# NVlabs/FasterViT

Hardware: AMD Instinct MI355X
Metric: images/sec FasterViT-0 224x224 inference, bs=256/GPU (higher is better)
Workload: dtype f16; 1 GPU; faster_vit_0_224 inference, 224x224, batch 256/GPU, synthetic weights (tests/synth.py init family); global_batch=256, parallelism=dp1 (independent shards, no data-path collective), hat_operands=f16, streams=1

## Files before the change

fastervit_amd/csrc/fvit_api.hip:

```cpp
#include <stdarg.h>
#include <stdlib.h>
#include <string.h>

#include <algorithm>
#include <map>
#include <mutex>
#include <string>
#include <vector>

#include "fvit_common.h"

namespace fvit {

static thread_local char g_err[512] = "";

void set_error(const char* fmt, ...) {
    va_list ap;
    va_start(ap, fmt);
    vsnprintf(g_err, sizeof(g_err), fmt, ap);
    va_end(ap);
}

int check_launch(const char* what) {
    hipError_t e = hipGetLastError();
// ... 170 lines not shown
                            const void* w_fc2_frag, const float* b_fc2, const float* gamma2, float eps) {
    return {dtype, X, rowsA, src_idx, add, R, batch, G, heads, C, hidden, ln1_w, ln1_b, w_qkv_frag, b_qkv_heads, w_proj_frag,
            b_proj, gamma1, bias, scale, ln2_w, ln2_b, w_fc1_frag, b_fc1, w_fc2_frag, b_fc2, gamma2, eps};
}

enum class CarrierRoute {
    NONE,
    FUSED_CT,
    ATTNBLK,
    LNGEMM_CHAIN,
    CHAIN,
};
enum class WinAttnRoute {
    WINBLK,
    ATTNBLK,
    LNGEMM_PREADDED,
    CHAIN,
};
enum class MlpRoute {
    WINMLP,
    MLP_FUSED,
    LNGEMM_CHAIN,
    CHAIN,
};

struct BlockRoute {
    CarrierRoute carrier = CarrierRoute::NONE;
    MlpRoute carrier_mlp = MlpRoute::CHAIN;
    WinAttnRoute window_attn = WinAttnRoute::CHAIN;
    MlpRoute window_mlp = MlpRoute::CHAIN;
    bool preadd_eligible = false;
    const float* pe_next = nullptr;
    int win_blk_split = 1, win_mlp_split = 1;
    RowMap entry_map;
    const float* entry_ct = nullptr;
    RowMap exit_map;
    const float* exit_ln_w = nullptr;
    const float* exit_ln_b = nullptr;
    float exit_eps = 0.f;
};

struct RouteKnobs {
    const int ln_gemm = tune_get("ln_gemm", 0), ln_gemm_max_rows = tune_get("ln_gemm_max_rows", 16384);
    const int attn_fused = tune_get("attn_fused", 1), attn_fused_x2 = tune_get("attn_fused_x2", 1);
    const int attn_fused_min_rows = tune_get("attn_fused_min_rows", 16384), attn_fused512_min_rows = tune_get("attn_fused512_min_rows", 1 << 30);
    const int mlp_fused = tune_get("mlp_fused", 1);
    const int mlp_fused_min_rows = tune_get("mlp_fused_min_rows", 16384), mlp_fused512_min_rows = tune_get("mlp_fused512_min_rows", 1 << 30);
    const int win_mlp = tune_get("win_mlp", 1), win_mlp256 = tune_get("win_mlp256", 2), win_mlp_split = tune_get("win_mlp_split", 1);
    const int win_fused = tune_get("win_fused", 1), win_fused256 = tune_get("win_fused256", 0), win_blk_split = tune_get("win_blk_split", 1);
    const int ct_fused = tune_get("ct_fused", 1), pe_preadd = tune_get("pe_preadd", 1);
    const int stage_entry_fused = tune_get("stage_entry_fused", 1), stage_exit_fused = tune_get("stage_exit_fused", 1);
};

static BlockRoute choose_route(const FvitStageDesc& d, const StageLayout& L, const FvitBlockWeights& w, const RouteKnobs& k) {
    const int T = d.weight_terms;
    auto ln_gemm_ok = [&](int N, int ldo, int64_t rows) {
        return T == 1 && ln_gemm_supported(d.C, N, L.ldn, ldo) && k.ln_gemm && rows <= k.ln_gemm_max_rows;
    };
    auto attnblk = [&](const FvitAttnWeights& a, int S, int64_t rows) {
        const bool terms_ok = T == 1 || (T == 2 && d.C == 256 && S > 48 && k.attn_fused_x2);
        return terms_ok && a.w_qkv_frag && a.b_qkv_heads && a.w_proj_frag && d.dpad == 32 && d.C / d.heads == 32 && attnblk_supported(d.C, d.heads, S) &&
               rows >= (d.C == 256 ? k.attn_fused_min_rows : k.attn_fused512_min_rows) && k.attn_fused;
    };
    auto mlp = [&](const FvitMlpWeights& m, int64_t rows) {
        const bool frags = m.w_fc1_frag && m.w_fc2_frag;
        if (T <= 2 && frags && winmlp_supported(d.C, d.hidden) && (d.C == 512 ? k.win_mlp != 0 : rows >= k.mlp_fused_min_rows && k.win_mlp256 != 0))
            return MlpRoute::WINMLP;
        if (T == 1 && frags && mlp_fused_supported(d.C, d.hidden) && rows >= (d.C == 256 ? k.mlp_fused_min_rows : k.mlp_fused512_min_rows) && k.mlp_fused)
            return MlpRoute::MLP_FUSED;
        return ln_gemm_ok(d.hidden, L.ldh, rows) ? MlpRoute::LNGEMM_CHAIN : MlpRoute::CHAIN;
    };

    BlockRoute r;
    r.win_blk_split = k.win_blk_split;
    r.win_mlp_split = k.win_mlp_split;
    if (d.hier) {
        const FvitAttnWeights& a = w.hat_attn;
        if (T <= 2 && ctblk_supported(d.C, d.heads, L.G, d.hidden) && d.dpad == 32 && a.w_qkv_frag && a.b_qkv_heads && a.w_proj_frag && a.bias &&
            w.hat_mlp.w_fc1_frag && w.hat_mlp.w_fc2_frag && k.ct_fused)
            r.carrier = CarrierRoute::FUSED_CT;
        else if (attnblk(a, L.G, L.Mc))
            r.carrier = CarrierRoute::ATTNBLK;
        else
            r.carrier = ln_gemm_ok(L.ldqkv, L.ldqkv, L.Mc) ? CarrierRoute::LNGEMM_CHAIN : CarrierRoute::CHAIN;
        r.carrier_mlp = mlp(w.hat_mlp, L.Mc);
    }
    const FvitAttnWeights& a = w.attn;
    if (T <= 2 && (T == 1 || d.C == 512) && winblk_supported(d.C, d.heads, L.S) && d.dpad == 32 && a.w_qkv_frag && a.b_qkv_heads && a.w_proj_frag && a.bias &&
        (d.C == 512 ? k.win_fused != 0 : k.win_fused256 != 0))
        r.window_attn = WinAttnRoute::WINBLK;
    else if (attnblk(a, L.S, L.Mx))
        r.window_attn = WinAttnRoute::ATTNBLK;
    r.window_mlp = mlp(w.mlp, L.Mx);
    r.preadd_eligible = !d.hier && r.window_attn == WinAttnRoute::CHAIN && (r.window_mlp == MlpRoute::CHAIN || r.window_mlp == MlpRoute::LNGEMM_CHAIN) &&
                        ln_gemm_ok(L.ldqkv, L.ldqkv, L.Mx) && k.pe_preadd;
    return r;
}

struct Branch {
    float* x;
    int64_t rows;
    void *xn, *qkv, *ao, *h;
    int nwin, S;
};

static LnCall ln_call(const FvitStageDesc& d, const StageLayout& L, const float* ln_w, const float* ln_b, const float* src, int64_t rows, void* n_out) {
    LnCall ln = {d.operand_dtype, src, 0, nullptr, 0, nullptr, nullptr, nullptr, nullptr, n_out, L.at * L.ldn, ln_w, ln_b, 1e-5f, (int)rows, 1, d.C};
    if (L.at == 2) ln.lo_off = L.ldn;
// ... 79 lines not shown
static AttnBlkCall window_attnblk_call(const FvitStageDesc& d, const StageLayout& L, const FvitBlockWeights& w, const FvitStageTables& t, float* X, float* R) {
    const FvitAttnWeights& a = w.attn;
    AttnBlkCall ab = attnblk_call(d.operand_dtype, X, L.rpi, R, L.G, (d.hier ? t.ln1_src : nullptr), t.ln1_add, w.pe_x, a.ln_w, a.ln_b, 1e-5f, L.rpi,
                                  a.w_qkv_frag, a.b_qkv_heads, a.w_proj_frag, a.b_proj, a.gamma, a.bias, X, d.batch * L.nW, L.S, d.heads, d.C, L.scale);
    ab.terms = d.weight_terms;
    return ab;
}

static MlpFusedCall window_mlp_call(const FvitStageDesc& d, const StageLayout& L, const FvitMlpWeights& w, float* X) {
    MlpFusedCall mc = mlp_fused_call(d.operand_dtype, X, (int)L.Mx, d.C, d.hidden, w.ln_w, w.ln_b, 1e-5f, w.w_fc1_frag, w.b_fc1, w.w_fc2_frag, w.b_fc2, w.gamma);
    mc.terms = d.weight_terms;
    return mc;
}

static RowMap row_map(const FvitStageDesc& d, const StageLayout& L, const FvitMapView& m) {
    RowMap r;
    r.data = m.data; r.stride_b = m.stride_b; r.stride_h = m.stride_h; r.stride_w = m.stride_w; r.bf16 = m.dtype == FVIT_BF16;
    r.S = L.S; r.ncw = L.ncw; r.ws = d.ws; r.nwx = d.Wp / d.ws; r.nw = L.nW;
    return r;
}
static bool map_16bit_cl(const FvitMapView& m, int align_bytes) {
    return (m.dtype == FVIT_F16 || m.dtype == FVIT_BF16) && m.stride_c == 1 && ((uintptr_t)m.data % align_bytes) == 0 && (m.stride_b * 2) % align_bytes == 0 &&
           (m.stride_h * 2) % align_bytes == 0 && (m.stride_w * 2) % align_bytes == 0;
}

static AttnBlkCall window_winblk_call(const FvitStageDesc& d, const StageLayout& L, const BlockRoute& r, const FvitBlockWeights& w, const FvitStageTables& t,
                                      float* X, float* R, char* ws) {
    AttnBlkCall ab = window_attnblk_call(d, L, w, t, X, R);
    if (L.off_SLAB) {
        ab.slab = (float*)(ws + L.off_SLAB);
        ab.counters = (int*)(ws + L.off_CNT);
        ab.nsplit = r.win_blk_split;
    }
    return ab;
}

static void choose_stage_boundaries(const FvitStageDesc& d, const StageLayout& L, const FvitBlockWeights* blocks, const FvitStageTables& t, const FvitMapView& in,
                                    const float* ct_init, const FvitMapView* out, const FvitStageTail* tail, bool prop, const ReverseCall& rc,
                                    const RouteKnobs& k, char* ws, std::vector<BlockRoute>& routes) {
    if (d.depth <= 0 || d.H != d.Hp || d.W != d.Wp || prop) return;
    for (int i = 0; i < d.depth; ++i)
        if (blocks[i].attn.gamma || blocks[i].mlp.gamma || (d.hier && (blocks[i].hat_attn.gamma || blocks[i].hat_mlp.gamma))) return;
    float* X = (float*)(ws + L.off_X);
    float* R = (float*)(ws + L.off_R);
    BlockRoute& first = routes[0];
    if (k.stage_entry_fused && map_16bit_cl(in, 8) && d.C % 4 == 0 && d.weight_terms <= 2) {
        bool ok = false;
        if (first.window_attn == WinAttnRoute::ATTNBLK) ok = attnblk_map_source_supported(window_attnblk_call(d, L, blocks[0], t, X, R));
        else if (first.window_attn == WinAttnRoute::WINBLK) ok = winblk_map_source_supported(window_winblk_call(d, L, first, blocks[0], t, X, R, ws));
        if (ok) {
            first.entry_map = row_map(d, L, in);
            if (first.carrier == CarrierRoute::FUSED_CT) first.entry_ct = ct_init;
        }
    }
    BlockRoute& last = routes[d.depth - 1];
    if (k.stage_exit_fused && tail && tail->ln_w && out && reverse_ln_supported(rc) && last.window_mlp == MlpRoute::WINMLP &&
        winmlp_exit_supported(window_mlp_call(d, L, blocks[d.depth - 1].mlp, X))) {
        last.exit_map = row_map(d, L, *out);
        last.exit_ln_w = tail->ln_w;
        last.exit_ln_b = tail->ln_b;
        last.exit_eps = tail->ln_eps;
    }
}

static int run_block(const FvitStageDesc& d, const StageLayout& L, const BlockRoute& r, const FvitBlockWeights& w, const FvitStageTables& t,
                     char* ws, hipStream_t st) {
// ... 385 lines not shown

int fvit_win_mlp_fused_terms(int32_t operand_dtype, float* x, int32_t M, int32_t C, int32_t hidden, const float* ln_w, const float* ln_b,
                             float eps, const void* w_fc1_frag, const float* b_fc1, const void* w_fc2_frag, const float* b_fc2,
                             const float* gamma, int32_t terms, fvit_stream_t stream) {
    MlpFusedCall mc = mlp_fused_call(operand_dtype, x, M, C, hidden, ln_w, ln_b, eps, w_fc1_frag, b_fc1, w_fc2_frag, b_fc2, gamma);
    mc.terms = terms;
    return launch_winmlp(mc, (hipStream_t)stream);
}

size_t fvit_win_mlp_split_bytes(int32_t M, int32_t C, int32_t nsplit) { return winmlp_split_slab_bytes(M, C, nsplit); }

int fvit_win_mlp_fused_split(int32_t operand_dtype, float* x, int32_t M, int32_t C, int32_t hidden, const float* ln_w, const float* ln_b,
                             float eps, const void* w_fc1_frag, const float* b_fc1, const void* w_fc2_frag, const float* b_fc2,
                             const float* gamma, int32_t terms, float* slab, int32_t* counters, int32_t nsplit, fvit_stream_t stream) {
    if (C != 512 || (nsplit != 1 && nsplit != 2) || (nsplit > 1 && (!slab || !counters))) {
        set_error("win_mlp_fused_split: C = %d nsplit = %d (C must be 512, nsplit 1 / 2 with scratch)", C, nsplit);
        return FVIT_EINVAL;
    }
    MlpFusedCall mc = mlp_fused_call(operand_dtype, x, M, C, hidden, ln_w, ln_b, eps, w_fc1_frag, b_fc1, w_fc2_frag, b_fc2, gamma);
    mc.terms = terms;
    mc.slab = slab; mc.counters = counters; mc.nsplit = nsplit;
    return launch_winmlp(mc, (hipStream_t)stream);
}

int fvit_win_block_supported(int32_t C, int32_t heads, int32_t S) { return winblk_supported(C, heads, S) ? 1 : 0; }

int fvit_win_block_fused(int32_t operand_dtype, const float* srcA, int32_t rowsA, const float* srcB, int32_t rowsB, const int32_t* src_idx,
                         const int32_t* add_idx, const float* add, const float* ln_w, const float* ln_b, float eps,
                         int32_t rows_per_image, const void* w_qkv_frag, const float* b_qkv_heads, const void* w_proj_frag,
                         const float* b_proj, const float* gamma, const float* bias, float* x_out, int32_t nwin, int32_t S,
                         int32_t heads, int32_t C, float scale, fvit_stream_t stream) {
    AttnBlkCall ab = attnblk_call(operand_dtype, srcA, rowsA, srcB, rowsB, src_idx, add_idx, add, ln_w, ln_b, eps, rows_per_image, w_qkv_frag,
                                  b_qkv_heads, w_proj_frag, b_proj, gamma, bias, x_out, nwin, S, heads, C, scale);
    return launch_winblk(ab, (hipStream_t)stream);
}

#ifdef FVIT_DIAG
int fvit_debug_win_mlp_timeline(float* x, int32_t M, int32_t C, int32_t hidden, const float* ln_w, const float* ln_b, float eps,
                                const void* w_fc1_frag, const float* b_fc1, const void* w_fc2_frag, const float* b_fc2, const float* gamma,
                                void* stamps, fvit_stream_t stream) {
    if (!stamps) { set_error("debug_win_mlp_timeline: null stamp buffer"); return FVIT_EINVAL; }
    MlpFusedCall mc = mlp_fused_call(FVIT_F16, x, M, C, hidden, ln_w, ln_b, eps, w_fc1_frag, b_fc1, w_fc2_frag, b_fc2, gamma);
    mc.ts = stamps;
    return launch_winmlp(mc, (hipStream_t)stream);
}
#endif

int fvit_win_block_fused_split(int32_t operand_dtype, const float* srcA, int32_t rowsA, const float* srcB, int32_t rowsB, const int32_t* src_idx,
                               const int32_t* add_idx, const float* add, const float* ln_w, const float* ln_b, float eps,
                               int32_t rows_per_image, const void* w_qkv_frag, const float* b_qkv_heads, const void* w_proj_frag,
                               const float* b_proj, const float* gamma, const float* bias, float* x_out, int32_t nwin, int32_t S,
                               int32_t heads, int32_t C, float scale, float* slab, int32_t* counters, int32_t nsplit, fvit_stream_t stream) {
    if (C != 512 || (nsplit != 1 && nsplit != 2) || (nsplit > 1 && (!slab || !counters))) {
        set_error("win_block_fused_split: C = %d nsplit = %d (C must be 512, nsplit 1 / 2 with scratch)", C, nsplit);
        return FVIT_EINVAL;
    }
    AttnBlkCall ab = attnblk_call(operand_dtype, srcA, rowsA, srcB, rowsB, src_idx, add_idx, add, ln_w, ln_b, eps, rows_per_image, w_qkv_frag,
                                  b_qkv_heads, w_proj_frag, b_proj, gamma, bias, x_out, nwin, S, heads, C, scale);
    ab.slab = slab; ab.counters = counters; ab.nsplit = nsplit;
    return launch_winblk(ab, (hipStream_t)stream);
}

int fvit_win_block_fused_terms(int32_t operand_dtype, const float* srcA, int32_t rowsA, const float* srcB, int32_t rowsB, const int32_t* src_idx,
                               const int32_t* add_idx, const float* add, const float* ln_w, const float* ln_b, float eps,
                               int32_t rows_per_image, const void* w_qkv_frag, const float* b_qkv_heads, const void* w_proj_frag,
                               const float* b_proj, const float* gamma, const float* bias, float* x_out, int32_t nwin, int32_t S,
                               int32_t heads, int32_t C, float scale, int32_t terms, fvit_stream_t stream) {
    AttnBlkCall ab = attnblk_call(operand_dtype, srcA, rowsA, srcB, rowsB, src_idx, add_idx, add, ln_w, ln_b, eps, rows_per_image, w_qkv_frag,
                                  b_qkv_heads, w_proj_frag, b_proj, gamma, bias, x_out, nwin, S, heads, C, scale);
    ab.terms = terms;
    return launch_winblk(ab, (hipStream_t)stream);
}

int fvit_attn_block_fused_terms(int32_t operand_dtype, const float* srcA, int32_t rowsA, const float* srcB, int32_t rowsB, const int32_t* src_idx,
                                const int32_t* add_idx, const float* add, const float* ln_w, const float* ln_b, float eps,
                                int32_t rows_per_image, const void* w_qkv_frag, const float* b_qkv_heads, const void* w_proj_frag,
                                const float* b_proj, const float* gamma, const float* bias, float* x_out, int32_t nwin, int32_t S,
                                int32_t heads, int32_t C, float scale, int32_t terms, fvit_stream_t stream) {
    AttnBlkCall ab = attnblk_call(operand_dtype, srcA, rowsA, srcB, rowsB, src_idx, add_idx, add, ln_w, ln_b, eps, rows_per_image, w_qkv_frag,
                                  b_qkv_heads, w_proj_frag, b_proj, gamma, bias, x_out, nwin, S, heads, C, scale);
    ab.terms = terms;
    return launch_attnblk(ab, (hipStream_t)stream);
}

int fvit_ct_block_supported(int32_t C, int32_t heads, int32_t G, int32_t hidden) { return ctblk_supported(C, heads, G, hidden) ? 1 : 0; }

int fvit_ct_block_fused(int32_t operand_dtype, const float* X, int32_t rowsA, const int32_t* src_idx, const float* add, float* R,
                        int32_t batch, int32_t G, int32_t heads, int32_t C, int32_t hidden, const float* ln1_w, const float* ln1_b,
                        const void* w_qkv_frag, const float* b_qkv_heads, const void* w_proj_frag, const float* b_proj, const float* gamma1,
                        const float* bias, float scale, const float* ln2_w, const float* ln2_b, const void* w_fc1_frag, const float* b_fc1,
                        const void* w_fc2_frag, const float* b_fc2, const float* gamma2, float eps, fvit_stream_t stream) {
    CtBlkCall cb = ctblk_call(operand_dtype, X, rowsA, src_idx, add, R, batch, G, heads, C, hidden, ln1_w, ln1_b, w_qkv_frag, b_qkv_heads, w_proj_frag,
                              b_proj, gamma1, bias, scale, ln2_w, ln2_b, w_fc1_frag, b_fc1, w_fc2_frag, b_fc2, gamma2, eps);
    return launch_ctblk(cb, (hipStream_t)stream);
}

int fvit_ct_block_fused_terms(int32_t operand_dtype, const float* X, int32_t rowsA, const int32_t* src_idx, const float* add, float* R,
                              int32_t batch, int32_t G, int32_t heads, int32_t C, int32_t hidden, const float* ln1_w, const float* ln1_b,
                              const void* w_qkv_frag, const float* b_qkv_heads, const void* w_proj_frag, const float* b_proj, const float* gamma1,
                              const float* bias, float scale, const float* ln2_w, const float* ln2_b, const void* w_fc1_frag, const float* b_fc1,
                              const void* w_fc2_frag, const float* b_fc2, const float* gamma2, float eps, int32_t terms, fvit_stream_t stream) {
    CtBlkCall cb = ctblk_call(operand_dtype, X, rowsA, src_idx, add, R, batch, G, heads, C, hidden, ln1_w, ln1_b, w_qkv_frag, b_qkv_heads, w_proj_frag,
                              b_proj, gamma1, bias, scale, ln2_w, ln2_b, w_fc1_frag, b_fc1, w_fc2_frag, b_fc2, gamma2, eps);
// ... 96 lines not shown
```

fastervit_amd/csrc/fvit_common.h:

```cpp
#pragma once
#include <hip/hip_runtime.h>
#include <stdint.h>
#include <atomic>
#include <mutex>
#include <stdio.h>

#include "../../include/fvit_hip.h"

namespace fvit {

typedef _Float16 h8 __attribute__((ext_vector_type(8)));
typedef _Float16 h4 __attribute__((ext_vector_type(4)));
typedef __bf16 b8 __attribute__((ext_vector_type(8)));
typedef __bf16 b4 __attribute__((ext_vector_type(4)));
typedef float f4 __attribute__((ext_vector_type(4)));

template <typename T> struct Op16;
template <> struct Op16<_Float16> {
    typedef h8 v8;
    typedef h4 v4;
    static __device__ __forceinline__ f4 mfma(v8 a, v8 b, f4 c) {
        return __builtin_amdgcn_mfma_f32_16x16x32_f16(a, b, c, 0, 0, 0);
    }
};
// ... 330 lines not shown
bool winmlp_exit_supported(const MlpFusedCall& c);
size_t winmlp_split_slab_bytes(int64_t M, int C, int nsplit);
bool mlp_fused_supported(int C, int hidden);
int launch_mlp_fused(const MlpFusedCall& c, hipStream_t stream);
bool winmlp_supported(int C, int hidden);
int launch_winmlp(const MlpFusedCall& c, hipStream_t stream);

struct AttnBlkCall {
    int dtype;
    const float* srcA;
    int rowsA;
    const float* srcB;
    int rowsB;
    const int32_t* src_idx;
    const int32_t* add_idx;
    const float* add;
    const float* ln_w;
    const float* ln_b;
    float eps;
    int rows_per_image;
    const void* wqkv_f;
    const float* bqkv;
    const void* wproj_f;
    const float* bproj;
    const float* gamma;
    const float* bias;
    float* x_out;
    int nwin, S, heads, C;
    float scale;
    float* slab = nullptr;
    int* counters = nullptr;
    int nsplit = 1;
    int terms = 1;
    void* ts = nullptr;
    RowMap map;
};
bool attnblk_supported(int C, int heads, int S);
bool attnblk_map_source_supported(const AttnBlkCall& c);
bool winblk_map_source_supported(const AttnBlkCall& c);
int launch_attnblk(const AttnBlkCall& c, hipStream_t stream);
bool attnblk2_supported(int C, int heads, int S);
int launch_attnblk2(const AttnBlkCall& c, hipStream_t stream);
bool winblk_supported(int C, int heads, int S);
int launch_winblk(const AttnBlkCall& c, hipStream_t stream);
struct AttnCall {
    int dtype;
    const void* qkv;
    int ldq;
    void* out;
    int ldo;
    const float* bias;
    int nwin, S, heads, dpad;
    float scale;
    const float* rel_table;
    int rel_w, rel_ng;
    int d;
    int q_lo_off = 0, o_lo_off = 0;
    const void* drop_mask = nullptr;
};
bool attention_dense(int S, int dpad);
int launch_attention(const AttnCall& c, hipStream_t stream);
int launch_attention_long(const AttnCall& c, hipStream_t stream);

struct LnCall {
    int dtype;
    const float* srcA;
// ... 81 lines not shown
```

fastervit_amd/csrc/fvit_winblk.hip:

```cpp
#include "fvit_common.h"

namespace fvit {

namespace {

struct WinBlkParams {
    const float* srcA;
    const float* srcB;
    const int32_t* src_idx;
    const int32_t* add_idx;
    const float* add;
    const float* ln_w;
    const float* ln_b;
    float eps;
    int rowsA, rowsB, rows_per_image;
    const void* wqkv_f;
    const float* bqkv;
    const void* wproj_f;
    const float* bproj;
    const float* gamma;
    const float* bias;
    float* x_out;
    int nwin, S;
    float scale;
    float* slab;
    int* counters;
    RowMap map;
};

template <int CC, int NSPLIT>
constexpr int winblk_lds_bytes() { return 4 * (CC / 32) * 1024 + 4 * (CC / 32 / NSPLIT) * 1024 + (CC / 32) * 96 * 4; }

template <typename T, int CC, int NWV, int NSPLIT = 1, int WT = 1, bool MAPSRC = false>
__device__ __forceinline__ void winblk_body(const WinBlkParams& p, char* const smem, const int blk) {
    typedef typename Op16<T>::v8 v8;
    constexpr int C = CC, KK = C / 32, CB = C / 16, HEADS = C / 32, NW = NWV, NRB = 4, SP = 64;
    constexpr int HW = HEADS / NSPLIT;
    constexpr int NH = HW / NW;
    static_assert(HW == NH * NW && NH >= 1 && CB == 4 * NW, "heads split evenly over the waves; four output channel blocks per wave");
    constexpr int KQ = KK * WT, PW = HW * WT;
    constexpr int SPH = KQ + 4;
    constexpr size_t QKV_IMG = (size_t)3 * C * C * 2, PROJ_IMG = (size_t)C * C * 2;
    constexpr int DEPTH = 2;
    constexpr int OFF_O = NRB * KK * 1024;
    constexpr int OFF_BQ = OFF_O + NRB * HW * 1024;
    static_assert(OFF_BQ + HEADS * 96 * 4 == winblk_lds_bytes<CC, NSPLIT>(), "LDS layout");
    float* bqs = (float*)(smem + OFF_BQ);

    const int tid = threadIdx.x;
    const int lane = tid & 63;
    const int wave = __builtin_amdgcn_readfirstlane(tid >> 6);
    const int g = lane >> 4, s = lane & 15;
    const int lane16 = lane * 16;
    int win = blk, sp = 0;
    if constexpr (NSPLIT > 1) {
        const int xcd = blk & 7, j = blk >> 3;
        win = (j / NSPLIT) * 8 + xcd;
        sp = j % NSPLIT;
        if (win >= p.nwin) return;
    }
    const int h0 = sp * HW;

    const char* Wq = (const char*)p.wqkv_f + lane16;
    const char* Wp = (const char*)p.wproj_f + lane16;
    const char* Bz = (const char*)p.bias + (s * SP + g * 4) * 4;
    v8 ring[DEPTH][6];
    auto load_qkv = [&](int slot, int h, int u) {
// ... 275 lines not shown
            const char* mpx = nullptr;
            if (p.src_idx) {
                const int si = p.src_idx[pr];
                src = si >= 0 ? p.srcA + ((size_t)b * p.rowsA + si) * C : p.srcB + ((size_t)b * p.rowsB + (-si - 1)) * C;
                if constexpr (MAPSRC) {
                    if (si >= 0) mpx = rowmap_px(p.map, (int64_t)b * p.rowsA + si);
                }
            } else {
                src = p.srcA + (size_t)row * C;
                if constexpr (MAPSRC) mpx = rowmap_px(p.map, row);
            }
            const int ai = p.add ? (p.add_idx ? p.add_idx[pr] : pr) : -1;
            float* px = p.x_out + (size_t)row * C + c0;
            f4 xm[4];
            if constexpr (MAPSRC) {
                if (mpx) rowmap_load_row(xm, mpx, p.map.bf16, [&](int q) { return c0 + q * 4; });
            }
#pragma unroll
            for (int q = 0; q < 4; ++q) {
                f4 xv;
                if (MAPSRC && mpx) xv = xm[q];
                else xv = *(const f4*)(src + c0 + q * 4);
                if (ai >= 0) xv += *(const f4*)(p.add + (size_t)ai * C + c0 + q * 4);
                const f4 bv = *(const f4*)(p.bproj + c0 + q * 4);
                const f4 gl = *(const f4*)((has_g ? p.gamma : p.bproj) + c0 + q * 4);
#pragma unroll
                for (int r = 0; r < 4; ++r) xv[r] += (has_g ? gl[r] : 1.f) * (oacc[q][rb][r] + bv[r]);
                *(f4*)(px + q * 4) = xv;
            }
        }
    }
}

template <typename T, int CC, int NWV, int NSPLIT = 1, int WT = 1, bool MAPSRC = false>
__global__ __launch_bounds__(64 * NWV, NWV == 8 ? 1 : 2) void winblk_kernel(WinBlkParams p) {
    __shared__ __attribute__((aligned(16))) char smem[winblk_lds_bytes<CC, NSPLIT>()];
    winblk_body<T, CC, NWV, NSPLIT, WT, MAPSRC>(p, smem, blockIdx.x);
}

inline WinBlkParams make_winblk_params(const AttnBlkCall& c) {
    WinBlkParams p;
    p.srcA = c.srcA; p.srcB = c.srcB; p.src_idx = c.src_idx; p.add_idx = c.add_idx; p.add = c.add; p.ln_w = c.ln_w; p.ln_b = c.ln_b; p.eps = c.eps;
    p.rowsA = c.rowsA; p.rowsB = c.rowsB; p.rows_per_image = c.rows_per_image > 0 ? c.rows_per_image : 1;
    p.wqkv_f = c.wqkv_f; p.bqkv = c.bqkv; p.wproj_f = c.wproj_f; p.bproj = c.bproj; p.gamma = c.gamma; p.bias = c.bias; p.x_out = c.x_out;
    p.nwin = c.nwin; p.S = c.S; p.scale = c.scale;
    p.slab = c.slab; p.counters = c.counters;
    p.map = c.map;
    return p;
}

}

#ifndef FVIT_BODIES_ONLY
bool winblk_supported(int C, int heads, int S) { return ((C == 512 && heads == 16) || (C == 256 && heads == 8)) && S > 48 && S <= 64; }

bool winblk_map_source_supported(const AttnBlkCall& c) {
    const bool split = c.C == 512 && c.terms == 1 && c.nsplit == 2 && c.slab && c.counters;
    return winblk_supported(c.C, c.heads, c.S) && !split && (c.terms == 1 || (c.terms == 2 && c.C == 512));
}

int launch_winblk(const AttnBlkCall& c, hipStream_t stream) {
    if (!winblk_supported(c.C, c.heads, c.S) || c.nwin <= 0 || !c.wqkv_f || !c.wproj_f || !c.x_out || !c.bias || !c.bqkv) {
        set_error("win_block: unsupported arguments C=%d heads=%d S=%d nwin=%d", c.C, c.heads, c.S, c.nwin);
        return FVIT_EINVAL;
    }
    if (ablate_skip(4)) return FVIT_OK;
    const WinBlkParams p = make_winblk_params(c);
    if (c.terms != 1 && !(c.terms == 2 && c.C == 512)) {
        set_error("win_block: weight terms %d with C = %d (two-term weights: C = 512 only)", c.terms, c.C);
        return FVIT_EINVAL;
    }
    const bool split = c.C == 512 && c.terms == 1 && c.nsplit == 2 && c.slab && c.counters;
    const double rows = (double)c.nwin * c.S;
    const double flops = rows * (2.0 * c.C * 3 * c.C + 4.0 * c.S * c.C + 2.0 * c.C * c.C);
    const bool mapsrc = c.map.data != nullptr;
    if (mapsrc && !winblk_map_source_supported(c)) {
        set_error("win_block: no map-source instance for C=%d terms=%d nsplit=%d", c.C, c.terms, c.nsplit);
        return FVIT_EINVAL;
    }
    const double bytes = rows * c.C * (mapsrc ? 6.0 : 8.0) + c.terms * 2.0 * 4.0 * c.C * c.C;
    ProfScope prof(FVIT_K_ATTN_FUSED, flops, bytes, stream);
    const int grid = split ? (c.nwin + 7) / 8 * 8 * 2 : c.nwin;
    prof_note(c.C == 512 ? (split ? "winblk_kernel<512,S64,split2>" : "winblk_kernel<512,S64>") : "winblk_kernel<256,S64>", grid);
    if (c.dtype != FVIT_F16 && c.dtype != FVIT_BF16) { set_error("win_block: operand dtype %d not supported", c.dtype); return FVIT_EINVAL; }
    if (mapsrc) {
#define FVIT_WB_MAP(T_) do { \
        if (c.terms == 2) hipLaunchKernelGGL((winblk_kernel<T_, 512, 8, 1, 2, true>), dim3(c.nwin), dim3(512), 0, stream, p); \
        else if (c.C == 512) hipLaunchKernelGGL((winblk_kernel<T_, 512, 8, 1, 1, true>), dim3(c.nwin), dim3(512), 0, stream, p); \
        else hipLaunchKernelGGL((winblk_kernel<T_, 256, 4, 1, 1, true>), dim3(c.nwin), dim3(256), 0, stream, p); } while (0)
        if (c.dtype == FVIT_F16) FVIT_WB_MAP(_Float16); else FVIT_WB_MAP(__bf16);
#undef FVIT_WB_MAP
    } else if (c.terms == 2) {
        if (c.dtype == FVIT_F16) hipLaunchKernelGGL((winblk_kernel<_Float16, 512, 8, 1, 2>), dim3(c.nwin), dim3(512), 0, stream, p);
        else hipLaunchKernelGGL((winblk_kernel<__bf16, 512, 8, 1, 2>), dim3(c.nwin), dim3(512), 0, stream, p);
    } else if (split) {
        if (c.dtype == FVIT_F16) hipLaunchKernelGGL((winblk_kernel<_Float16, 512, 8, 2>), dim3(grid), dim3(512), 0, stream, p);
        else hipLaunchKernelGGL((winblk_kernel<__bf16, 512, 8, 2>), dim3(grid), dim3(512), 0, stream, p);
    } else if (c.C == 512) {
        if (c.dtype == FVIT_F16) hipLaunchKernelGGL((winblk_kernel<_Float16, 512, 8>), dim3(c.nwin), dim3(512), 0, stream, p);
        else hipLaunchKernelGGL((winblk_kernel<__bf16, 512, 8>), dim3(c.nwin), dim3(512), 0, stream, p);
    } else {
        if (c.dtype == FVIT_F16) hipLaunchKernelGGL((winblk_kernel<_Float16, 256, 4>), dim3(c.nwin), dim3(256), 0, stream, p);
        else hipLaunchKernelGGL((winblk_kernel<__bf16, 256, 4>), dim3(c.nwin), dim3(256), 0, stream, p);
    }
    return check_launch("winblk_kernel");
}

#endif

}
```

Measured before the change: 94110 images/s.

## Add register-ring weight prefetch variant of the C=512 fused window-attention block

Adds a new body for the C=512 unsplit window-attention kernel, on by default through a new tuning knob. It streams QKV weights, relative-position bias and projection weights through a three-deep register ring, so global loads are issued ahead of the MFMAs that consume them. It also caches per-token source descriptors in LDS and restructures the LayerNorm and residual handling. The cost is extra LDS and register pressure on a one-block-per-CU kernel, which could lower occupancy or cause spills.

```diff
diff --git a/fastervit_amd/csrc/fvit_api.hip b/fastervit_amd/csrc/fvit_api.hip
--- a/fastervit_amd/csrc/fvit_api.hip
+++ b/fastervit_amd/csrc/fvit_api.hip
@@ -226,6 +226,7 @@
     bool preadd_eligible = false;
     const float* pe_next = nullptr;
     int win_blk_split = 1, win_mlp_split = 1;
+    int win_blk_form = 1;
     RowMap entry_map;
     const float* entry_ct = nullptr;
     RowMap exit_map;
@@ -243,6 +244,7 @@
     const int win_mlp = tune_get("win_mlp", 1), win_mlp256 = tune_get("win_mlp256", 2), win_mlp_split = tune_get("win_mlp_split", 1);
     const int win_fused = tune_get("win_fused", 1), win_fused256 = tune_get("win_fused256", 0), win_blk_split = tune_get("win_blk_split", 1);
     const int ct_fused = tune_get("ct_fused", 1), pe_preadd = tune_get("pe_preadd", 1);
+    const int win_blk_form = tune_get("win_blk_form", 1);
     const int stage_entry_fused = tune_get("stage_entry_fused", 1), stage_exit_fused = tune_get("stage_exit_fused", 1);
 };
 
@@ -268,6 +270,7 @@
     BlockRoute r;
     r.win_blk_split = k.win_blk_split;
     r.win_mlp_split = k.win_mlp_split;
+    r.win_blk_form = k.win_blk_form;
     if (d.hier) {
         const FvitAttnWeights& a = w.hat_attn;
         if (T <= 2 && ctblk_supported(d.C, d.heads, L.G, d.hidden) && d.dpad == 32 && a.w_qkv_frag && a.b_qkv_heads && a.w_proj_frag && a.bias &&
@@ -413,6 +416,7 @@
         ab.counters = (int*)(ws + L.off_CNT);
         ab.nsplit = r.win_blk_split;
     }
+    ab.form = r.win_blk_form;
     return ab;
 }
 
@@ -864,6 +868,7 @@
                          int32_t heads, int32_t C, float scale, fvit_stream_t stream) {
     AttnBlkCall ab = attnblk_call(operand_dtype, srcA, rowsA, srcB, rowsB, src_idx, add_idx, add, ln_w, ln_b, eps, rows_per_image, w_qkv_frag,
                                   b_qkv_heads, w_proj_frag, b_proj, gamma, bias, x_out, nwin, S, heads, C, scale);
+    ab.form = tune_get("win_blk_form", 1);
     return launch_winblk(ab, (hipStream_t)stream);
 }
 
@@ -901,6 +906,7 @@
     AttnBlkCall ab = attnblk_call(operand_dtype, srcA, rowsA, srcB, rowsB, src_idx, add_idx, add, ln_w, ln_b, eps, rows_per_image, w_qkv_frag,
                                   b_qkv_heads, w_proj_frag, b_proj, gamma, bias, x_out, nwin, S, heads, C, scale);
     ab.terms = terms;
+    ab.form = tune_get("win_blk_form", 1);
     return launch_winblk(ab, (hipStream_t)stream);
 }
 
diff --git a/fastervit_amd/csrc/fvit_common.h b/fastervit_amd/csrc/fvit_common.h
--- a/fastervit_amd/csrc/fvit_common.h
+++ b/fastervit_amd/csrc/fvit_common.h
@@ -386,6 +386,7 @@
     int* counters = nullptr;
     int nsplit = 1;
     int terms = 1;
+    int form = 1;
     void* ts = nullptr;
     RowMap map;
 };
diff --git a/fastervit_amd/csrc/fvit_winblk.hip b/fastervit_amd/csrc/fvit_winblk.hip
--- a/fastervit_amd/csrc/fvit_winblk.hip
+++ b/fastervit_amd/csrc/fvit_winblk.hip
@@ -31,8 +31,430 @@
 template <int CC, int NSPLIT>
 constexpr int winblk_lds_bytes() { return 4 * (CC / 32) * 1024 + 4 * (CC / 32 / NSPLIT) * 1024 + (CC / 32) * 96 * 4; }
 
-template <typename T, int CC, int NWV, int NSPLIT = 1, int WT = 1, bool MAPSRC = false>
+constexpr int FORM1_DEPTH = 3;
+constexpr int FORM1_EXTRA_LDS = 4 * 512 * 4 + 64 * 16;
+
+template <typename T, int WT, bool MAPSRC>
+__device__ __forceinline__ void winblk_body_form1(const WinBlkParams& p, char* const smem, const int blk) {
+    typedef typename Op16<T>::v8 v8;
+    typedef float f2 __attribute__((ext_vector_type(2)));
+    typedef float f4a8 __attribute__((ext_vector_type(4), aligned(8)));
+    constexpr int C = 512, KK = C / 32, CB = C / 16, HEADS = C / 32, NW = 8, NRB = 4, SP = 64, NH = HEADS / NW;
+    constexpr int KQ = KK * WT, KV = KQ / 2, PW = HEADS * WT;
+    constexpr int SPH = KQ + KV + 4;
+    constexpr size_t QKV_IMG = (size_t)3 * C * C * 2, PROJ_IMG = (size_t)C * C * 2;
+    constexpr int DEPTH = FORM1_DEPTH, PRE = 2;
+    constexpr int OFF_O = NRB * KK * 1024, OFF_BQ = OFF_O + NRB * HEADS * 1024, OFF_BP = winblk_lds_bytes<C, 1>();
+    static_assert(OFF_BQ + HEADS * 96 * 4 == OFF_BP, "LDS layout");
+    static_assert(2 * NRB * NW * 64 * 16 <= NRB * HEADS * 1024, "the row statistics of phase A fit in the O region");
+    float* const bqs = (float*)(smem + OFF_BQ);
+    float* const bps = (float*)(smem + OFF_BP);
+
+    const int tid = threadIdx.x;
+    const int lane = tid & 63;
+    const int wave = __builtin_amdgcn_readfirstlane(tid >> 6);
+    const int g = lane >> 4, s = lane & 15;
+    const int lane16 = lane * 16;
+    const int win = blk;
+    const int c0 = wave * 64 + g * 16;
+
+    const char* Wq = (const char*)p.wqkv_f + lane16;
+    const char* Wp = (const char*)p.wproj_f + lane16;
+    const char* Bz = (const char*)p.bias + (s * SP + g * 4) * 4;
+    auto zero = []() { int z = 0; asm volatile("" : "+v"(z)); return z; };
+    v8 ring[DEPTH][4];
+    auto issue = [&](int t) {
+        const int slot = t % DEPTH;
+        if (t < NH * SPH) {
+            const int hh = t / SPH, u = t - hh * SPH, h = NH * wave + hh;
+            if (u < KQ) {
+                const char* base = Wq + (u / KK) * QKV_IMG + ((size_t)h * 6 * KK + u % KK) * 1024;
+#pragma unroll
+                for (int ub = 0; ub < 4; ++ub) ring[slot][ub] = *(const v8*)(base + (size_t)ub * KK * 1024);
+            } else if (u < KQ + KV) {
+                const int u0 = 2 * (u - KQ);
+                const char* base = Wq + (u0 / KK) * QKV_IMG + (((size_t)h * 6 + 4) * KK + u0 % KK) * 1024;
+#pragma unroll
+                for (int i = 0; i < 4; ++i) ring[slot][i] = *(const v8*)(base + ((size_t)(i & 1) * KK + (i >> 1)) * 1024);
+            } else {
+                const int qb = u - KQ - KV;
+#pragma unroll
+                for (int kb = 0; kb < 4; ++kb) ring[slot][kb] = *(const v8*)(Bz + ((size_t)(h * SP + qb * 16) * SP + kb * 16) * 4);
+            }
+        } else if (t < NH * SPH + PW) {
+            const int hp = t - NH * SPH;
+            const char* base = Wp + (hp / HEADS) * PROJ_IMG + ((size_t)(hp % HEADS) * CB + 4 * wave) * 1024;
+#pragma unroll
+            for (int q = 0; q < 4; ++q) ring[slot][q] = *(const v8*)(base + q * 1024);
+        }
+        __builtin_amdgcn_sched_barrier(0);
+    };
+    struct TokDesc { const char* ptr; int ai; int from_map; };
+    static_assert(sizeof(TokDesc) == 16, "one ds_read_b128 per token");
+    TokDesc* const tds = (TokDesc*)(smem + OFF_BP + 4 * C * 4);
+    const uint32_t trow = (uint32_t)win * p.S + (lane < p.S ? lane : p.S - 1);
+    const int tb = (int)(trow / (uint32_t)p.rows_per_image), tpr = (int)(trow - (uint32_t)tb * p.rows_per_image);
+    int tsi = 0, tai = -1;
+    if (wave == 0) {
+        if (p.src_idx) tsi = p.src_idx[tpr];
+        if (p.add) tai = p.add_idx ? p.add_idx[tpr] : tpr;
+    }
+    __builtin_amdgcn_sched_barrier(0);
+#pragma unroll
+    for (int t = 0; t < PRE; ++t) issue(t);
+    if (wave == 0) {
+        const float* src;
+        const char* mpx = nullptr;
+        if (p.src_idx) {
+            src = tsi >= 0 ? p.srcA + ((size_t)tb * p.rowsA + tsi) * C : p.srcB + ((size_t)tb * p.rowsB + (-tsi - 1)) * C;
+            if constexpr (MAPSRC) {
+                if (tsi >= 0) mpx = rowmap_px(p.map, (int64_t)tb * p.rowsA + tsi);
+            }
+        } else {
+            src = p.srcA + (size_t)trow * C;
+            if constexpr (MAPSRC) mpx = rowmap_px(p.map, trow);
+        }
+        TokDesc d;
+        d.ptr = mpx ? mpx : (const char*)src;
+        d.ai = tai;
+        d.from_map = mpx != nullptr;
+        tds[lane] = d;
+    }
+    __syncthreads();
+    TokDesc td[NRB];
+#pragma unroll
+    for (int rb = 0; rb < NRB; ++rb) td[rb] = tds[rb * 16 + s];
+#define GLOBAL_AS __attribute__((address_space(1)))
+    auto request_row = [&](f4 (&x)[4], const TokDesc& d) {
+        if (MAPSRC && d.from_map) {
+            x[0] = *(const GLOBAL_AS f4a8*)(d.ptr + 2 * c0);
+            x[1] = *(const GLOBAL_AS f4a8*)(d.ptr + 2 * c0 + 16);
+        } else {
+#pragma unroll
+            for (int q = 0; q < 4; ++q) x[q] = *(const GLOBAL_AS f4*)(d.ptr + 4 * (c0 + q * 4));
+        }
+    };
+#undef GLOBAL_AS
+    auto widen_row = [&](f4 (&x)[4], const TokDesc& d) {
+        if (MAPSRC && d.from_map) {
+            const f4 r0 = x[0], r1 = x[1];
+#pragma unroll
+            for (int q = 0; q < 4; ++q) {
+                const f4 rr = q < 2 ? r0 : r1;
+                const f2 raw = {rr[2 * (q & 1)], rr[2 * (q & 1) + 1]};
+                if (p.map.bf16) {
+                    const b4 hv = __builtin_bit_cast(b4, raw);
+#pragma unroll
+                    for (int r = 0; r < 4; ++r) x[q][r] = (float)hv[r];
+                } else {
+                    const h4 hv = __builtin_bit_cast(h4, raw);
+#pragma unroll
+                    for (int r = 0; r < 4; ++r) x[q][r] = (float)hv[r];
+                }
+            }
+        }
+    };
+
+    {
+        f4 v[NRB][4];
+#pragma unroll
+        for (int rb = 0; rb < NRB; ++rb) request_row(v[rb], td[rb]);
+        if (p.add) {
+            f4 a[NRB][4];
+#pragma unroll
+            for (int rb = 0; rb < NRB; ++rb) {
+                const float* addp = p.add + (size_t)(td[rb].ai >= 0 ? td[rb].ai : 0) * C + c0;
+#pragma unroll
+                for (int q = 0; q < 4; ++q) a[rb][q] = *(const f4*)(addp + q * 4);
+            }
+            __builtin_amdgcn_sched_barrier(0);
+#pragma unroll
+            for (int rb = 0; rb < NRB; ++rb) {
+                widen_row(v[rb], td[rb]);
+#pragma unroll
+                for (int q = 0; q < 4; ++q)
+#pragma unroll
+                    for (int r = 0; r < 4; ++r) v[rb][q][r] += td[rb].ai >= 0 ? a[rb][q][r] : 0.f;
+            }
+        } else {
+            __builtin_amdgcn_sched_barrier(0);
+#pragma unroll
+            for (int rb = 0; rb < NRB; ++rb) {
+                widen_row(v[rb], td[rb]);
+#pragma unroll
+                for (int q = 0; q < 4; ++q)
+#pragma unroll
+                    for (int r = 0; r < 4; ++r) v[rb][q][r] += 0.f;
+            }
+        }
+        float cbq[HEADS * 96 / (64 * NW)];
+#pragma unroll
+        for (int i = 0; i < HEADS * 96 / (64 * NW); ++i) cbq[i] = p.bqkv[tid + 64 * NW * i];
+        const float cbp = p.bproj[tid], cgm = p.gamma ? p.gamma[tid] : 1.f, clw = p.ln_w[tid], clb = p.ln_b[tid];
+        __builtin_amdgcn_sched_barrier(0);
+        f4* const part = (f4*)(smem + OFF_O + lane16 + zero());
+        float mean[NRB], rstd[NRB];
+#pragma unroll
+        for (int rb = 0; rb < NRB; ++rb) {
+            f4 t;
+#pragma unroll
+            for (int q = 0; q < 4; ++q) t[q] = (v[rb][q][0] + v[rb][q][1]) + (v[rb][q][2] + v[rb][q][3]);
+            part[(rb * NW + wave) * 64] = t;
+        }
+        __syncthreads();
+#pragma unroll
+        for (int i = 0; i < HEADS * 96 / (64 * NW); ++i) bqs[tid + 64 * NW * i] = cbq[i];
+        bps[tid] = cbp;
+        bps[C + tid] = cgm;
+        bps[2 * C + tid] = clw;
+        bps[3 * C + tid] = clb;
+#pragma unroll
+        for (int rb = 0; rb < NRB; ++rb) {
+            float sum = 0.f;
+#pragma unroll
+            for (int w = 0; w < NW; ++w) {
+                const f4 t = part[(rb * NW + w) * 64];
+#pragma unroll
+                for (int q = 0; q < 4; ++q) sum += t[q];
+            }
+            sum = sum_xor32(sum_xor16(sum));
+            mean[rb] = sum / (float)C;
+            f4 t;
+#pragma unroll
+            for (int q = 0; q < 4; ++q) {
+                const f4 d = v[rb][q] - mean[rb];
+                t[q] = (d[0] * d[0] + d[1] * d[1]) + (d[2] * d[2] + d[3] * d[3]);
+            }
+            part[((NRB + rb) * NW + wave) * 64] = t;
+            __builtin_amdgcn_sched_barrier(0);
+        }
+        __syncthreads();
+#pragma unroll
+        for (int rb = 0; rb < NRB; ++rb) {
+            float sq = 0.f;
+#pragma unroll
+            for (int w = 0; w < NW; ++w) {
+                const f4 t = part[((NRB + rb) * NW + w) * 64];
+#pragma unroll
+                for (int q = 0; q < 4; ++q) sq += t[q];
+            }
+            sq = sum_xor32(sum_xor16(sq));
+            rstd[rb] = rsqrtf(sq / (float)C + p.eps);
+            __builtin_amdgcn_sched_barrier(0);
+        }
+#pragma unroll
+        for (int t = PRE; t < DEPTH; ++t) issue(t);
+        f4 lnw[4], lnb[4];
+#pragma unroll
+        for (int q = 0; q < 4; ++q) {
+            lnw[q] = *(const f4*)(bps + 2 * C + c0 + q * 4);
+            lnb[q] = *(const f4*)(bps + 3 * C + c0 + q * 4);
+        }
+#pragma unroll
+        for (int rb = 0; rb < NRB; ++rb)
+#pragma unroll
+            for (int k2 = 0; k2 < 2; ++k2) {
+                v8 o;
+#pragma unroll
+                for (int h2 = 0; h2 < 2; ++h2)
+#pragma unroll
+                    for (int r = 0; r < 4; ++r)
+                        o[h2 * 4 + r] = sat16<T>((v[rb][2 * k2 + h2][r] - mean[rb]) * rstd[rb] * lnw[2 * k2 + h2][r] + lnb[2 * k2 + h2][r]);
+                *(v8*)(smem + ((rb * KK + 2 * wave + k2) * 1024) + lane16) = o;
+            }
+    }
+    __syncthreads();
+
+    const char* xn = smem + lane16;
+#pragma unroll
+    for (int hh = 0; hh < NH; ++hh) {
+        const int h = NH * wave + hh;
+        const float* bq = bqs + h * 96;
+        {
+            const int z = zero();
+            Wq += z;
+            Bz += z;
+            if (hh == NH - 1) Wp += z;
+        }
+        v8 qf[NRB], kf[NRB], vf[2][2];
+        {
+            f4 acc[4][NRB];
+#pragma unroll
+            for (int ub = 0; ub < 4; ++ub)
+#pragma unroll
+                for (int rb = 0; rb < NRB; ++rb) acc[ub][rb] = (f4){0.f, 0.f, 0.f, 0.f};
+#pragma unroll
+            for (int u = 0; u < KQ; ++u) {
+                const int t = hh * SPH + u, kk = u % KK;
+                v8 xb[NRB];
+#pragma unroll
+                for (int rb = 0; rb < NRB; ++rb) xb[rb] = *(const v8*)(xn + (rb * KK + kk) * 1024);
+#pragma unroll
+                for (int ub = 0; ub < 4; ++ub)
+#pragma unroll
+                    for (int rb = 0; rb < NRB; ++rb) acc[ub][rb] = Op16<T>::mfma(ring[t % DEPTH][ub], xb[rb], acc[ub][rb]);
+                __builtin_amdgcn_sched_barrier(0);
+                issue(t + DEPTH);
+            }
+#pragma unroll
+            for (int blk2 = 0; blk2 < 2; ++blk2) {
+                const f4 bqv = *(const f4*)(bq + blk2 * 16 + g * 4);
+                const f4 bkv = *(const f4*)(bq + 32 + blk2 * 16 + g * 4);
+#pragma unroll
+                for (int rb = 0; rb < NRB; ++rb)
+#pragma unroll
+                    for (int r = 0; r < 4; ++r) {
+                        qf[rb][blk2 * 4 + r] = sat16<T>(acc[blk2][rb][r] + bqv[r]);
+                        kf[rb][blk2 * 4 + r] = sat16<T>(acc[2 + blk2][rb][r] + bkv[r]);
+                    }
+                __builtin_amdgcn_sched_barrier(0);
+            }
+        }
+        {
+            f4 av[2][NRB];
+#pragma unroll
+            for (int db = 0; db < 2; ++db)
+#pragma unroll
+                for (int rb = 0; rb < NRB; ++rb) av[db][rb] = (f4){0.f, 0.f, 0.f, 0.f};
+#pragma unroll
+            for (int j = 0; j < KV; ++j) {
+                const int t = hh * SPH + KQ + j;
+#pragma unroll
+                for (int e = 0; e < 2; ++e) {
+                    const int kk = (2 * j + e) % KK;
+                    v8 xb[NRB];
+#pragma unroll
+                    for (int rb = 0; rb < NRB; ++rb) xb[rb] = *(const v8*)(xn + (rb * KK + kk) * 1024);
+#pragma unroll
+                    for (int db = 0; db < 2; ++db)
+#pragma unroll
+                        for (int rb = 0; rb < NRB; ++rb) av[db][rb] = Op16<T>::mfma(xb[rb], ring[t % DEPTH][2 * e + db], av[db][rb]);
+                }
+                __builtin_amdgcn_sched_barrier(0);
+                issue(t + DEPTH);
+            }
+#pragma unroll
+            for (int db = 0; db < 2; ++db) {
+                const float bv = bq[64 + db * 16 + s];
+#pragma unroll
+                for (int k32 = 0; k32 < 2; ++k32)
+#pragma unroll
+                    for (int r = 0; r < 4; ++r) {
+                        vf[db][k32][r] = sat16<T>(av[db][2 * k32][r] + bv);
+                        vf[db][k32][4 + r] = sat16<T>(av[db][2 * k32 + 1][r] + bv);
+                    }
+            }
+        }
+#pragma unroll
+        for (int qb = 0; qb < NRB; ++qb) {
+            const int t = hh * SPH + KQ + KV + qb;
+            f4 sc[NRB];
+            float mx = -3.0e38f;
+#pragma unroll
+            for (int kb = 0; kb < NRB; ++kb) {
+                f4 a = Op16<T>::mfma(kf[kb], qf[qb], (f4){0.f, 0.f, 0.f, 0.f});
+                const f4 bz = __builtin_bit_cast(f4, ring[t % DEPTH][kb]);
+#pragma unroll
+                for (int r = 0; r < 4; ++r) {
+                    a[r] = a[r] * p.scale + bz[r];
+                    mx = fmaxf(mx, a[r]);
+                }
+                sc[kb] = a;
+            }
+            __builtin_amdgcn_sched_barrier(0);
+            issue(t + DEPTH);
+            mx = max_xor32(max_xor16(mx));
+            float sum = 0.f;
+#pragma unroll
+            for (int kb = 0; kb < NRB; ++kb)
+#pragma unroll
+                for (int r = 0; r < 4; ++r) {
+                    const float e = __expf(sc[kb][r] - mx);
+                    sc[kb][r] = e;
+                    sum += e;
+                }
+            sum = sum_xor32(sum_xor16(sum));
+            const float inv = 1.0f / sum;
+            f4 o[2] = {(f4){0.f, 0.f, 0.f, 0.f}, (f4){0.f, 0.f, 0.f, 0.f}};
+#pragma unroll
+            for (int k32 = 0; k32 < 2; ++k32) {
+                v8 pf;
+#pragma unroll
+                for (int r = 0; r < 4; ++r) {
+                    pf[r] = (T)sc[2 * k32][r];
+                    pf[4 + r] = (T)sc[2 * k32 + 1][r];
+                }
+#pragma unroll
+                for (int db = 0; db < 2; ++db) o[db] = Op16<T>::mfma(vf[db][k32], pf, o[db]);
+            }
+            v8 of;
+#pragma unroll
+            for (int r = 0; r < 4; ++r) {
+                of[r] = sat16<T>(o[0][r] * inv);
+                of[4 + r] = sat16<T>(o[1][r] * inv);
+            }
+            *(v8*)(smem + OFF_O + ((qb * HEADS + h) * 1024) + lane16) = of;
+        }
+    }
+    __syncthreads();
+
+    Wp += zero();
+    const char* const xo = xn + OFF_O + zero();
+    f4 oacc[4][NRB], xr[NRB][4], ar[NRB][4];
+#pragma unroll
+    for (int q = 0; q < 4; ++q)
+#pragma unroll
+        for (int rb = 0; rb < NRB; ++rb) oacc[q][rb] = (f4){0.f, 0.f, 0.f, 0.f};
+#pragma unroll
+    for (int hp = 0; hp < PW; ++hp) {
+        const int t = NH * SPH + hp, h = hp % HEADS;
+        v8 ob[NRB];
+#pragma unroll
+        for (int rb = 0; rb < NRB; ++rb) ob[rb] = *(const v8*)(xo + (rb * HEADS + h) * 1024);
+#pragma unroll
+        for (int q = 0; q < 4; ++q)
+#pragma unroll
+            for (int rb = 0; rb < NRB; ++rb) oacc[q][rb] = Op16<T>::mfma(ring[t % DEPTH][q], ob[rb], oacc[q][rb]);
+        __builtin_amdgcn_sched_barrier(0);
+        issue(t + DEPTH);
+        if (hp >= PW - NRB && p.add) {
+            const int rb = hp - (PW - NRB), ai = tds[rb * 16 + s].ai;
+            const float* addp = p.add + (size_t)(ai >= 0 ? ai : 0) * C + c0;
+#pragma unroll
+            for (int q = 0; q < 4; ++q) ar[rb][q] = *(const f4*)(addp + q * 4);
+            __builtin_amdgcn_sched_barrier(0);
+        }
+    }
+
+#pragma unroll
+    for (int rb = 0; rb < NRB; ++rb) {
+        const int tok = rb * 16 + s;
+        const TokDesc d = tds[tok];
+        request_row(xr[rb], d);
+        widen_row(xr[rb], d);
+        if (tok < p.S) {
+            float* px = p.x_out + ((size_t)win * p.S + tok) * C + c0;
+#pragma unroll
+            for (int q = 0; q < 4; ++q) {
+                f4 xv = xr[rb][q];
+                if (d.ai >= 0) xv += ar[rb][q];
+                const f4 bv = *(const f4*)(bps + c0 + q * 4);
+                const f4 gl = *(const f4*)(bps + C + c0 + q * 4);
+#pragma unroll
+                for (int r = 0; r < 4; ++r) xv[r] += gl[r] * (oacc[q][rb][r] + bv[r]);
+                *(f4*)(px + q * 4) = xv;
+            }
+        }
+    }
+}
+
+template <typename T, int CC, int NWV, int NSPLIT = 1, int WT = 1, bool MAPSRC = false, int FORM = 0>
 __device__ __forceinline__ void winblk_body(const WinBlkParams& p, char* const smem, const int blk) {
+    if constexpr (FORM == 1) {
+        static_assert(CC == 512 && NWV == 8 && NSPLIT == 1, "FORM 1: the C = 512, 8-wave, unsplit instances");
+        winblk_body_form1<T, WT, MAPSRC>(p, smem, blk);
+        return;
+    }
     typedef typename Op16<T>::v8 v8;
     constexpr int C = CC, KK = C / 32, CB = C / 16, HEADS = C / 32, NW = NWV, NRB = 4, SP = 64;
     constexpr int HW = HEADS / NSPLIT;
@@ -374,10 +796,10 @@
     }
 }
 
-template <typename T, int CC, int NWV, int NSPLIT = 1, int WT = 1, bool MAPSRC = false>
+template <typename T, int CC, int NWV, int NSPLIT = 1, int WT = 1, bool MAPSRC = false, int FORM = 0>
 __global__ __launch_bounds__(64 * NWV, NWV == 8 ? 1 : 2) void winblk_kernel(WinBlkParams p) {
-    __shared__ __attribute__((aligned(16))) char smem[winblk_lds_bytes<CC, NSPLIT>()];
-    winblk_body<T, CC, NWV, NSPLIT, WT, MAPSRC>(p, smem, blockIdx.x);
+    __shared__ __attribute__((aligned(16))) char smem[winblk_lds_bytes<CC, NSPLIT>() + (FORM == 1 ? FORM1_EXTRA_LDS : 0)];
+    winblk_body<T, CC, NWV, NSPLIT, WT, MAPSRC, FORM>(p, smem, blockIdx.x);
 }
 
 inline WinBlkParams make_winblk_params(const AttnBlkCall& c) {
@@ -425,26 +847,29 @@
     const int grid = split ? (c.nwin + 7) / 8 * 8 * 2 : c.nwin;
     prof_note(c.C == 512 ? (split ? "winblk_kernel<512,S64,split2>" : "winblk_kernel<512,S64>") : "winblk_kernel<256,S64>", grid);
     if (c.dtype != FVIT_F16 && c.dtype != FVIT_BF16) { set_error("win_block: operand dtype %d not supported", c.dtype); return FVIT_EINVAL; }
+    const bool form1 = c.form == 1 && c.C == 512 && !split;
+#define FVIT_WB_512(T_, WT_, MAP_) do { \
+        if (form1) hipLaunchKernelGGL((winblk_kernel<T_, 512, 8, 1, WT_, MAP_, 1>), dim3(c.nwin), dim3(512), 0, stream, p); \
+        else hipLaunchKernelGGL((winblk_kernel<T_, 512, 8, 1, WT_, MAP_, 0>), dim3(c.nwin), dim3(512), 0, stream, p); } while (0)
     if (mapsrc) {
 #define FVIT_WB_MAP(T_) do { \
-        if (c.terms == 2) hipLaunchKernelGGL((winblk_kernel<T_, 512, 8, 1, 2, true>), dim3(c.nwin), dim3(512), 0, stream, p); \
-        else if (c.C == 512) hipLaunchKernelGGL((winblk_kernel<T_, 512, 8, 1, 1, true>), dim3(c.nwin), dim3(512), 0, stream, p); \
+        if (c.terms == 2) FVIT_WB_512(T_, 2, true); \
+        else if (c.C == 512) FVIT_WB_512(T_, 1, true); \
         else hipLaunchKernelGGL((winblk_kernel<T_, 256, 4, 1, 1, true>), dim3(c.nwin), dim3(256), 0, stream, p); } while (0)
         if (c.dtype == FVIT_F16) FVIT_WB_MAP(_Float16); else FVIT_WB_MAP(__bf16);
 #undef FVIT_WB_MAP
     } else if (c.terms == 2) {
-        if (c.dtype == FVIT_F16) hipLaunchKernelGGL((winblk_kernel<_Float16, 512, 8, 1, 2>), dim3(c.nwin), dim3(512), 0, stream, p);
-        else hipLaunchKernelGGL((winblk_kernel<__bf16, 512, 8, 1, 2>), dim3(c.nwin), dim3(512), 0, stream, p);
+        if (c.dtype == FVIT_F16) FVIT_WB_512(_Float16, 2, false); else FVIT_WB_512(__bf16, 2, false);
     } else if (split) {
         if (c.dtype == FVIT_F16) hipLaunchKernelGGL((winblk_kernel<_Float16, 512, 8, 2>), dim3(grid), dim3(512), 0, stream, p);
         else hipLaunchKernelGGL((winblk_kernel<__bf16, 512, 8, 2>), dim3(grid), dim3(512), 0, stream, p);
     } else if (c.C == 512) {
-        if (c.dtype == FVIT_F16) hipLaunchKernelGGL((winblk_kernel<_Float16, 512, 8>), dim3(c.nwin), dim3(512), 0, stream, p);
-        else hipLaunchKernelGGL((winblk_kernel<__bf16, 512, 8>), dim3(c.nwin), dim3(512), 0, stream, p);
+        if (c.dtype == FVIT_F16) FVIT_WB_512(_Float16, 1, false); else FVIT_WB_512(__bf16, 1, false);
     } else {
         if (c.dtype == FVIT_F16) hipLaunchKernelGGL((winblk_kernel<_Float16, 256, 4>), dim3(c.nwin), dim3(256), 0, stream, p);
         else hipLaunchKernelGGL((winblk_kernel<__bf16, 256, 4>), dim3(c.nwin), dim3(256), 0, stream, p);
     }
+#undef FVIT_WB_512
     return check_launch("winblk_kernel");
 }
 
```

After: 94750 images/s, median of 6. About the same (+0.7%).
